# walaj/SeqLib

Measured on AMD Instinct MI355X. Metric: aligned reads/sec (150 bp) via BWAAligner, higher is better.
Workload: dtype int32

## Files before the change

### seqlib_amd/csrc/dev_fin.h

```cpp
#pragma once
#include "dev_ext.h"
#include "dev_as.h"

#define DEV_MINUS_INF (-0x40000000)

template <typename QF, typename TF>
__device__ int dev_ksw_global2(int qlen, QF qf, int tlen, TF tf, const slx_opt &o, int w, uint8_t *z, int n_col, int *eh_h, int *eh_e)
{
    const int8_t *mat = o.mat;
    const int o_del = o.o_del, e_del = o.e_del, o_ins = o.o_ins, e_ins = o.e_ins;
    const int oe_del = o_del + e_del, oe_ins = o_ins + e_ins;
    int i, j;
    eh_h[0] = 0; eh_e[0] = DEV_MINUS_INF;
    for (j = 1; j <= qlen && j <= w; ++j) { eh_h[j] = -(o_ins + e_ins * j); eh_e[j] = DEV_MINUS_INF; }
    for (; j <= qlen; ++j) eh_h[j] = eh_e[j] = DEV_MINUS_INF;
    for (i = 0; i < tlen; ++i) {
        int f = DEV_MINUS_INF, h1, beg, end, t;
        const int8_t *qrow = mat + tf(i) * 5;
        beg = i > w ? i - w : 0;
        end = i + w + 1 < qlen ? i + w + 1 : qlen;
        h1 = beg == 0 ? -(o_del + e_del * (i + 1)) : DEV_MINUS_INF;
        uint8_t *zi = z ? z + (size_t)i * n_col : nullptr;
        for (j = beg; j < end; ++j) {
            int h, m = eh_h[j], e = eh_e[j];
// ... 310 lines not shown
        const int64_t l_pac = rfl_i64(R.l_pac);
        SortStage S;
        S.idx = S.ka = S.kb = S.m_qe = S.m_rid = S.m_w = nullptr; S.k64 = S.m_rb = nullptr; S.nmax = 0; S.lane = 0;
        if (ss) {
            S.idx = lds_uniform(ss->idx); S.k64 = lds_uniform(ss->k64); S.ka = lds_uniform(ss->ka); S.kb = lds_uniform(ss->kb);
            S.m_rb = lds_uniform(ss->m_rb); S.m_qe = lds_uniform(ss->m_qe); S.m_rid = lds_uniform(ss->m_rid); S.m_w = lds_uniform(ss->m_w);
            S.nmax = rfl_i32(ss->nmax); S.lane = ss->lane;
            n = rfl_i32(n);
        }
        const bool staged = ss != nullptr && n <= S.nmax && n >= 2;
        glb_ptr<DReg> Gg = as_glb(G);
        glb_ptr<int> ag = as_glb(a);
        if (staged) { Gg = as_glb_uniform(G); ag = as_glb_uniform(a); }
        const bool dbg = ck.dbg_cyc && ck.dbg_stage == 2;
        unsigned long long t0 = dbg ? __builtin_readcyclecounter() : 0ull, t1 = t0, t2 = t0, t3 = t0;
        auto sort_handles = [&](int m, auto fill, auto less_lds, auto less_glb) {
            if (!staged) { ks_introsort_idx(m, a, less_glb); return; }
            __threadfence_block();
            for (int i = S.lane; i < m; i += 64) { const int h = ag[i]; S.idx[i] = h; fill(h); }
            fin_sync<MAXQ>();
            bool tie = m > 768;
            if (!tie) for (int e = S.lane; e < m; e += 64) {
                const int he = S.idx[e];
                int rank = 0;
                for (int j = 0; j < m; ++j) {
                    const int hj = S.idx[j];
                    const bool lt = less_lds(hj, he);
                    rank += lt ? 1 : 0;
                    if (!lt && j != e && !less_lds(he, hj)) tie = true;
                }
                S.m_w[e] = rank;
            }
            if (!__any(tie)) {
                fin_sync<MAXQ>();
                for (int e = S.lane; e < m; e += 64) S.m_rid[S.m_w[e]] = S.idx[e];
                fin_sync<MAXQ>();
                for (int e = S.lane; e < m; e += 64) { const int h = S.m_rid[e]; S.idx[e] = h; ag[e] = h; }
            } else {
                fin_sync<MAXQ>();
                if (S.lane == 0) ks_introsort_idx(m, S.idx, less_lds);
                fin_sync<MAXQ>();
                for (int i = S.lane; i < m; i += 64) ag[i] = S.idx[i];
            }
            fin_sync<MAXQ>();
            __threadfence_block();
        };
        if (staged) { for (int i = S.lane; i < n; i += 64) ag[i] = i; __threadfence_block(); }
        else for (int i = 0; i < n; ++i) a[i] = i;
        if (n > 1) {
            sort_handles(n, [&](int h) { S.k64[h] = Gg[h].re; },
                         [&](int x, int y) { return S.k64[x] < S.k64[y]; },
                         [&](int x, int y) { return G[x].re < G[y].re; });
            if (dbg) t1 = __builtin_readcyclecounter();
            if (defer && !staged && n <= 64) {
                for (int i = 1; i < n; ++i) {
                    const DReg &p = G[a[i]];
                    if (p.rid != G[a[i - 1]].rid || p.rb >= G[a[i - 1]].re + opt.max_chain_gap) continue;
                    for (int j = i - 1; j >= 0 && p.rid == G[a[j]].rid && p.rb < G[a[j]].re + opt.max_chain_gap; --j) {
                        const DReg &q = G[a[j]];
                        if (q.rb < p.rb && dev_patch_pre(R, opt, q.rb, q.re, q.qb, q.qe, q.w, p.rb, p.re, p.qb, p.qe, p.w) >= 0) { *defer = true; return -1; }
                    }
                }
            }
            if (staged) { for (int i = S.lane; i < n; i += 64) Gg[i].n_comp = 1; __threadfence_block(); }
            else for (int i = 0; i < n; ++i) G[a[i]].n_comp = 1;
// ... 111 lines not shown
                    const int i = base + S.lane;
                    const int h = i < n_in ? S.idx[i] : 0;
                    const bool keep = i < n_in && (i < first_forced || S.m_qe[h] > S.kb[h]);
                    const unsigned long long km = __ballot(keep);
                    const int pos = m + (int)__builtin_amdgcn_mbcnt_hi((uint32_t)(km >> 32), __builtin_amdgcn_mbcnt_lo((uint32_t)km, 0u));
                    if (keep) ag[pos] = h;
                    m += (int)__popcll(km);
                }
                __threadfence_block();
                return m;
            };
            int m = 0;
            if (staged) m = compact_staged(n, 0);
            else for (int i = 0; i < n; ++i) if (G[a[i]].qe > G[a[i]].qb) a[m++] = a[i];
            n = m;
            sort_handles(n, [&](int h) { S.ka[h] = Gg[h].score; S.k64[h] = Gg[h].rb; S.kb[h] = Gg[h].qb; },
                         [&](int x, int y) {
                             const int sx = S.ka[x], sy = S.ka[y];
                             const int64_t bx = S.k64[x], by = S.k64[y];
                             return sx > sy || (sx == sy && (bx < by || (bx == by && S.kb[x] < S.kb[y])));
                         },
                         [&](int x, int y) {
                             const DReg &X = G[x], &Y = G[y];
                             return X.score > Y.score || (X.score == Y.score && (X.rb < Y.rb || (X.rb == Y.rb && X.qb < Y.qb)));
                         });
            if (staged) {
                for (int i = 1 + S.lane; i < n; i += 64) {
                    const int h = S.idx[i], hp = S.idx[i - 1];
                    if (S.ka[h] == S.ka[hp] && S.k64[h] == S.k64[hp] && S.kb[h] == S.kb[hp]) { Gg[h].qe = S.kb[h]; S.m_qe[h] = S.kb[h]; }
                }
                fin_sync<MAXQ>();
// ... 65 lines not shown
                int n_pri = 0;
                for (int base = 0; base < n; base += 64) {
                    const int i = base + lane;
                    bool pri = false;
                    if (i < n) {
                        const int h = ag[i];
                        const glb_ptr<DReg> p = Gg + h;
                        p->sub = 0; p->secondary = -1; p->hash = dev_hash_64(id + (uint64_t)i);
                        const int al = ref_is_alt(R, p->rid);
                        l_alt[h] = al;
                        pri = !al;
                    }
                    n_pri += (int)__popcll(__ballot(pri));
                }
                __threadfence_block();
                sort_handles(n, [&](int h) { S.ka[h] = Gg[h].score; S.k64[h] = (int64_t)Gg[h].hash; },
                             [&](int x, int y) {
                                 const int sx = S.ka[x], sy = S.ka[y];
                                 if (sx != sy) return sx > sy;
                                 const int ax = l_alt[x], ay = l_alt[y];
                                 return ax < ay || (ax == ay && (uint64_t)S.k64[x] < (uint64_t)S.k64[y]);
                             },
                             [&](int x, int y) { return false; });
                core_staged(n, l_alt);
                if (n_pri < n) {
                    for (int i = lane; i < n; i += 64) { const int h = S.idx[i], sidx = Gg[h].secondary; l_par[h] = sidx >= 0 ? S.idx[sidx] : -1; }
                    fin_sync<MAXQ>();
                    if (n_pri > 0)
                        sort_handles(n, [&](int h) { S.ka[h] = Gg[h].score; S.k64[h] = (int64_t)Gg[h].hash; },
                                     [&](int x, int y) {
                                         const int ax = l_alt[x], ay = l_alt[y];
                                         if (ax != ay) return ax < ay;
                                         const int sx = S.ka[x], sy = S.ka[y];
                                         return sx > sy || (sx == sy && (uint64_t)S.k64[x] < (uint64_t)S.k64[y]);
                                     },
                                     [&](int x, int y) { return false; });
                    const lds_ptr<int> l_rank = (lds_ptr<int>)S.k64;
                    fin_sync<MAXQ>();
                    for (int i = lane; i < n; i += 64) l_rank[S.idx[i]] = i;
                    fin_sync<MAXQ>();
                    for (int i = lane; i < n; i += 64) {
                        const int h = S.idx[i], ph = l_par[h];
                        if (ph >= 0) { par[h] = l_rank[ph]; if (l_alt[h]) Gg[h].secondary = 0x7fffffff; }
                        else par[h] = -1;
// ... 5 lines not shown
                } else
                    for (int i = lane; i < n; i += 64) { const int h = S.idx[i]; par[h] = Gg[h].secondary; }
                __threadfence_block();
                fin_sync<MAXQ>();
            } else if (R.ann_alt) {
                dev_mark_primary_alt(R, opt, w, n, id);
            } else {
            if (staged) {
                for (int i = S.lane; i < n; i += 64) { const glb_ptr<DReg> p = Gg + ag[i]; p->sub = 0; p->secondary = -1; p->hash = dev_hash_64(id + (uint64_t)i); }
                __threadfence_block();
            } else for (int i = 0; i < n; ++i) {
                DReg &p = G[a[i]];
                p.sub = 0; p.secondary = -1;
                p.hash = dev_hash_64(id + (uint64_t)i);
            }
            sort_handles(n, [&](int h) { S.ka[h] = Gg[h].score; S.k64[h] = (int64_t)Gg[h].hash; },
                         [&](int x, int y) {
                             const int sx = S.ka[x], sy = S.ka[y];
                             return sx > sy || (sx == sy && (uint64_t)S.k64[x] < (uint64_t)S.k64[y]);
                         },
                         [&](int x, int y) {
                             const DReg &X = G[x], &Y = G[y];
                             return X.score > Y.score || (X.score == Y.score && X.hash < Y.hash);
                         });
            if (staged) core_staged(n, nullptr);
            else {
            int *z = w.ib, nz = 0;
            z[nz++] = 0;
            for (int i = 1; i < n; ++i) {
                int k;
                DReg &ai = G[a[i]];
// ... 67 lines not shown
```

### seqlib_amd/csrc/dev_fin2.h

```cpp
#pragma once
#include "dev_fin.h"
#include "dev_ext_reg.h"
#include "dev_nm8.h"

#ifndef LANE_CIG_BAND
#define LANE_CIG_BAND 33
#endif
#define LANE_CIG_MAXQ 158
#define LANE_CIG_MAXT 400
#define LANE_NEG (-16000)
#define LANE_FIN_LIMIT 8000
static_assert(LANE_NEG + LANE_FIN_LIMIT <= -LANE_FIN_LIMIT && LANE_NEG >= -32768 && LANE_FIN_LIMIT <= 32767, "16-bit cells of k_cig_lanes");
#define LANE_IL_WORDS(max_len) (((LANE_CIG_BAND + 3) / 4) * (((max_len) < LANE_CIG_MAXQ ? (max_len) : LANE_CIG_MAXQ) + 16))
struct alignas(8) DJob {
    int64_t rb, re;
    int qb, qe;
    int w2, truesc;
    int r, pad;
};

struct FinLists {
    DJob *jobs;
    uint32_t *fast_list, *dp_list;
    unsigned int *n_fast, *n_dp, *q_dp;
// ... 348 lines not shown
    __shared__ SortTables<NB> tables;
    const int lane = threadIdx.x;
    const SortStage ss = tables.stage(lane);
    const MatRows mr = make_matrows(dopt.o.mat);
    const int n_todo = __builtin_amdgcn_readfirstlane((int)*n_slots);
    for (;;) {
        const int slot = (int)wave_take(queue, 1u);
        if (slot >= n_todo) break;
        const int r = order ? order[slot] : slot;
        const int nr = __builtin_amdgcn_readfirstlane(ck.n_reg[r]);
        const bool mine = nr >= min_regs && nr <= max_regs;
        if (mine) dev_regs_read_wave<MAXQ>(R, ck, dopt.o, mr, fl, r, lane, &ss);
#ifdef REGS_SLEEP
        if (mine && nr >= 256) for (int t = 0; t < REGS_SLEEP; ++t) __builtin_amdgcn_s_sleep(127);
#endif
    }
}

__device__ __forceinline__ void dev_finish_hit(const DevRef &R, const Chunk &ck, const DJob &j, int l_query, DHit &h, int64_t cs, int nc)
{
    int is_rev;
    int64_t pos = dev_depos(R, j.rb < R.l_pac ? j.rb : j.re - 1, &is_rev);
    if (nc > 0) {
        if ((ck.cigpool[cs] & 0xf) == 2) { pos += ck.cigpool[cs] >> 4; ++cs; --nc; }
        else if ((ck.cigpool[cs + nc - 1] & 0xf) == 2) --nc;
    }
    if (j.qb != 0 || j.qe != l_query) {
        const int clip5 = is_rev ? l_query - j.qe : j.qb, clip3 = is_rev ? j.qb : l_query - j.qe;
        const uint32_t cop = ck.hardclip ? 5u : 4u;
        if (clip5) { --cs; ck.cigpool[cs] = (uint32_t)clip5 << 4 | cop; ++nc; }
// ... 253 lines not shown
    if (blockIdx.x < (n_jobs + CIG_BATCH - 1) / CIG_BATCH) {
        const unsigned long long off = wave_take_u64(ck.zused, (unsigned long long)CIG_WAVE_Z);
        if (off + CIG_WAVE_Z <= ck.zcap) { ws.z_own = ck.zarena + off; ws.z_own_cap = CIG_WAVE_Z; }
        else if (lane == 0) atomicOr(ck.flags + 1, OVS_Z_DP_WAVE);
    }
    for (;;) {
        const unsigned int t0 = wave_take(fl.q_dp, (unsigned int)CIG_BATCH);
        if (t0 >= n_jobs) break;
        const unsigned int t1 = t0 + CIG_BATCH < n_jobs ? t0 + CIG_BATCH : n_jobs;
        for (unsigned int t = t0; t < t1; ++t) dev_cig_dp_job<MAXQ>(R, ck, dopt.o, mr, fl, fl.dp_list[t], lane, ws);
    }
}

#define HITS_BIG 12
#define HITS_WAVE_N 2048
__global__ void __launch_bounds__(64) k_hits_wave(Chunk ck, const int *list, const unsigned int *n_list, unsigned int *queue)
{
    __shared__ int64_t s_pos[HITS_WAVE_N];
    __shared__ int s_rid[HITS_WAVE_N], s_mapq[HITS_WAVE_N];
    const int lane = threadIdx.x;
    const int n_todo = __builtin_amdgcn_readfirstlane((int)*n_list);
    for (;;) {
        const int slot = (int)wave_take(queue, 1u);
        if (slot >= n_todo) break;
        const int r = list[slot];
        ReadWS w = make_ws(ck, r);
        const int nh = __builtin_amdgcn_readfirstlane(ck.n_hit[r]);
        int *hh = w.ic;
        auto less_glb = [&](int x, int y) {
            const DHit &A = w.hits[x], &B = w.hits[y];
            if (A.mapq != B.mapq) return A.mapq > B.mapq;
            if (A.rid != B.rid) return A.rid < B.rid;
            return A.pos < B.pos;
        };
        bool serial = nh > HITS_WAVE_N;
        if (!serial) {
            __syncthreads();
            for (int e = lane; e < nh; e += 64) { const DHit &h = w.hits[e]; s_pos[e] = h.pos; s_rid[e] = h.rid; s_mapq[e] = h.mapq; }
            __syncthreads();
            bool tie = false;
            for (int base = 0; base < nh; base += 64) {
                const int e = base + lane;
                const bool live = e < nh;
                const int em = live ? s_mapq[e] : 0, er = live ? s_rid[e] : 0;
                const int64_t ep = live ? s_pos[e] : 0;
                int rank = 0;
                for (int j = 0; j < nh; ++j) {
                    const int jm = s_mapq[j], jr = s_rid[j];
                    const int64_t jp = s_pos[j];
                    const bool lt = jm != em ? jm > em : (jr != er ? jr < er : jp < ep);
                    rank += lt ? 1 : 0;
                    if (live && j != e && jm == em && jr == er && jp == ep) tie = true;
                }
                if (live) hh[rank] = e;
            }
            serial = __any(tie) != 0;
        }
        __threadfence_block();
        if (serial) {
            if (lane == 0) {
                for (int i = 0; i < nh; ++i) hh[i] = i;
                std_sort_idx(nh, hh, less_glb);
            }
            __threadfence_block();
        }
        __syncthreads();
        int n_out = 0;
        double carry = 0;
        for (int base = 0; base < nh; base += 64) {
            const int i = base + lane;
            const bool live = i < nh;
            const int hi = live ? hh[i] : 0;
            int flag = 0, score = 0;
// ... 115 lines not shown
```

### seqlib_amd/csrc/dev_types.h

```cpp
#pragma once
#include <hip/hip_runtime.h>
#include <stdint.h>
#include "seqlib_amd.h"
#include "dev_wave.h"

enum : uint32_t {
    OVF_INTV = 1u << 0,
    OVF_LIST = 1u << 1,
    OVF_ZARENA = 1u << 2,
    OVF_CIGAR = 1u << 3,
    ERR_LOGLUT = 1u << 4,
    ERR_INTERNAL = 1u << 5,
};
enum : uint32_t {
    OVS_Z_GEN = 1u << 8,
    OVS_Z_BAND = 1u << 9,
    OVS_Z_BAND_BLOCK = 1u << 10,
    OVS_Z_SEG = 1u << 11,
    OVS_Z_LANE = 1u << 12,
    OVS_Z_DP = 1u << 13,
    OVS_Z_DP_WAVE = 1u << 14,
    OVS_C_BAND = 1u << 15,
    OVS_C_LANE = 1u << 16,
    OVS_C_LONG = 1u << 17,
// ... 81 lines not shown
    int32_t *s_next;
    int32_t *s_score;
    int64_t *c_pos;
    int32_t *c_head, *c_tail, *c_n, *c_rid, *c_w, *c_first;
    int8_t *c_kept;
    int32_t *ia, *ib, *ic;
    uint64_t *srt;
    DReg *regs;
    DHit *hits;
    const DReg *cand;
    const int32_t *cand_base;
    unsigned long long *dbg_cyc;
    int dbg_stage;
    int ext_row_exit;
    unsigned int *ext_exits;
    int32_t *n_chain;
    int32_t *n_reg;
    int32_t *n_hit;
    int32_t *na;
    float *frac_rep;
    uint8_t *zarena; unsigned long long zcap; unsigned long long *zused;
    uint32_t *cigpool; unsigned long long cigcap; unsigned long long *cigused;
    const double *log_lut; int log_lut_n;
    uint32_t *flags;
    void *lists; int cap_list; int n_threads;
    int *long_scratch; int long_stride; int long_threads;
    int *huge_rows; int huge_stride;
    int hardclip; double keepSecFrac; int maxSecondary;
    int sam_mode;
};
// ... 54 lines not shown
```

### seqlib_amd/csrc/slx_align.hip

```cpp
#include <hip/hip_runtime.h>
#include <hipcub/hipcub.hpp>
#include <chrono>
#include <cmath>
#include <functional>
#include <unistd.h>
#include <cstdio>
#include <cstdlib>
#include <cstring>
#include <algorithm>
#include <mutex>
#include <string>
#include <thread>
#include <type_traits>
#include <vector>
#include "slx_internal.h"
#include "dev_seed4.h"
#include "dev_fin.h"
#include "dev_ext_wave.h"
#include "dev_ext_reg.h"
#include "dev_ext_lane.h"
#include "dev_ext_block.h"
#include "dev_ext_seg.h"
#include "dev_fin2.h"
#include "dev_chain_coop.h"
// ... 475 lines not shown
        while ((int)al->workers.size() < (int)value) { const int rc = add_worker(al); if (rc != SLX_OK) return rc; }
        al->n_workers = (int)value;
    }
    else if (!strcmp(key, "min_split")) { if (value < 1) return SLX_EINVAL; al->min_split = value; }
    else if (!strcmp(key, "seed_quota")) { if (value < 0 || value > (1 << 24)) return SLX_EINVAL; al->seed_quota = (int)value; }
    else if (!strcmp(key, "rep_k")) {
        if (value < 0 || value > 31) return SLX_EINVAL;
        al->rep_k = (int)value;
        HIPCHK(hipSetDevice(al->device));
        return al->wide ? build_rep_filter<uint64_t>(al) : build_rep_filter<uint32_t>(al);
    }
    else if (!strcmp(key, "top_heavy")) al->top_heavy = value != 0;
    else if (!strcmp(key, "top_reuse")) al->top_reuse = value != 0;
    else if (!strcmp(key, "walk_stage")) al->walk_stage = value != 0;
    else if (!strcmp(key, "ext_row_exit")) al->ext_row_exit = value != 0;
    else if (!strcmp(key, "ext_narrow")) { if (value < 0 || value > 3) return SLX_EINVAL; al->ext_narrow = (int)value; }
    else if (!strcmp(key, "p2_items")) al->p2_items = value != 0;
    else if (!strcmp(key, "p2_coop")) al->p2_coop = value != 0;
    else if (!strcmp(key, "p2_items_cap")) al->p2_items_cap = (int)value;
    else if (!strcmp(key, "seed_free_cus")) {
        if (value < 0 || value > 24) return SLX_EINVAL;
        HIPCHK(hipSetDevice(al->device));
        al->seed_free_cus = (int)value;
        for (Worker *wk : al->workers) { const int rc = set_seed_stream(al, wk); if (rc != SLX_OK) return rc; }
    }
    else if (!strcmp(key, "stream_prio")) {
        if (value < 0 || value > 1) return SLX_EINVAL;
        HIPCHK(hipSetDevice(al->device));
        al->stream_prio = (int)value;
        for (Worker *wk : al->workers) {
// ... 72 lines not shown
            long long v = 0;
            auto take = [&](const slx_aligner *a) { for (const Worker *wk : a->workers) v += (long long)wk->first_stat; };
            if (al->is_group) for (const slx_aligner *sub : al->subs) take(sub); else take(al);
            return v;
        }
        if (!strcmp(key, "ext_narrow_sides") || !strcmp(key, "ext_narrow_jobs")) {
            long long v = 0;
            const int which = key[11] == 'j';
            auto take = [&](const slx_aligner *a) { for (const Worker *wk : a->workers) v += (long long)wk->narrow_stat[which]; };
            if (al->is_group) for (const slx_aligner *sub : al->subs) take(sub); else take(al);
            return v;
        }
        if (!strcmp(key, "walk_staged_chains")) {
            long long v = 0;
            auto take = [&](const slx_aligner *a) { for (const Worker *wk : a->workers) v += (long long)wk->walk_stat; };
            if (al->is_group) for (const slx_aligner *sub : al->subs) take(sub); else take(al);
            return v;
        }
        if (!strcmp(key, "ext_row_exits")) {
            long long v = 0;
            auto take = [&](const slx_aligner *a) { for (const Worker *wk : a->workers) v += (long long)wk->exit_stat; };
            if (al->is_group) for (const slx_aligner *sub : al->subs) take(sub); else take(al);
            return v;
        }
        if (!strcmp(key, "retries")) {
            long long v = 0;
            if (al->is_group) for (const slx_aligner *sub : al->subs) v += sub->n_retries; else v = al->n_retries;
            return v;
        }
        if (!strcmp(key, "ovf_sites")) {
// ... 103 lines not shown
    if (h_offs && r_hi > r_lo) {
        const uint64_t b0 = h_offs[r_lo], b1 = h_offs[r_hi];
        if (b0 < al->h_first || b1 < b0 || b1 > al->h_last) { slx_set_error("read offsets are not monotonic (part [%lld, %lld))", (long long)r_lo, (long long)r_hi); return SLX_EINVAL; }
        if (b1 > b0) HIPCHK(hipMemcpyAsync((void *)(d_bases + b0), h_bases + b0, b1 - b0, hipMemcpyHostToDevice, wk->stream));
        HIPCHK(hipMemcpyAsync((void *)(d_offs + r_lo), h_offs + r_lo, ((size_t)(r_hi - r_lo) + 1) * 8, hipMemcpyHostToDevice, wk->stream));
    }
    for (int i = 0; i < SLX_N_STAGES; ++i) wk->stage_ms[i] = 0;
    for (int i = 0; i < SLX_N_PROBES; ++i) wk->probe_ms[i] = 0;
    wk->n_chunks = 0;
    for (long long &c : wk->cnt) c = 0;
    wk->chain_stat[0] = wk->chain_stat[1] = 0;
    wk->first_stat = 0;
    wk->walk_stat = 0;
    wk->exit_stat = 0;
    wk->narrow_stat[0] = wk->narrow_stat[1] = 0;
    int rc;
    const int64_t n_part = r_hi - r_lo;
    if ((rc = wk->o_hit_off.ensure(((size_t)n_part + 1) * 8)) != SLX_OK) return rc;
    if ((rc = wk->len_stat.ensure(32)) != SLX_OK) return rc;
    int64_t hit_base = 0, cig_base = 0;
    for (int64_t r0 = r_lo, step = 0; r0 < r_hi; r0 += step) {
        const int n = (int)std::min<int64_t>(al->chunk_reads, r_hi - r0);
        step = n;
        unsigned long long stat[4] = {0, 0, 0, 0};
        HIPCHK(hipMemsetAsync(wk->len_stat.p, 0, 32, wk->stream));
        hipLaunchKernelGGL(k_len_stats, dim3((unsigned)((n + 255) / 256)), dim3(256), 0, wk->stream, d_offs + r0, n, wk->len_stat.as<unsigned long long>());
        { MailSpec ms{}; ms.src[0] = wk->len_stat.as<unsigned int>(); ms.words[0] = 8; ms.n = 1;
          hipLaunchKernelGGL(k_mail, dim3(1), dim3(64), 0, wk->stream, ms, wk->h_mail); }
        HIPCHK(slx_wait_stream(wk->stream));
        memcpy(stat, wk->h_mail, 32);
// ... 581 lines not shown
```

### seqlib_amd/csrc/slx_align_types.h

```cpp
#pragma once
#include <hip/hip_runtime.h>
#include <mutex>
#include <string>
#include <vector>
#include "slx_internal.h"
#include "slx_hip.h"
#include "dev_fm.h"
#include "dev_types.h"

#define HIPCHK(x) SLX_HIPCHK(x)

struct DevBuf : SlxDevBuf<SlxMargin<8, 256>> {
    int grow(size_t bytes, size_t keep, hipStream_t st) { return bytes <= cap ? SLX_OK : slx_dev_realloc(&p, &cap, SlxMargin<2, 256>::want(bytes), st, keep); }
};

#define SLX_MAIL_PARTS 8
struct MailSpec { const unsigned int *src[SLX_MAIL_PARTS]; int words[SLX_MAIL_PARTS]; int n; };
static __global__ void k_mail(MailSpec s, unsigned int *dst)
{
    int at = 0;
    for (int i = 0; i < s.n; ++i) {
        for (int w = (int)threadIdx.x; w < s.words[i]; w += (int)blockDim.x) dst[at + w] = s.src[i][w];
        at += s.words[i];
    }
// ... 20 lines not shown
    DevBuf p2mask, p2list, p2items, p2long, lane_jobs, first_dp, cig_lane_list;
    DevBuf job_key_in, job_key_out, job_val_in, job_val_out, job_sort_tmp;
    DevBuf seed3_buf;
    DevBuf memo_idx, memo_jobs, memo_tab, round_list, todo_a, todo_b, spec_cnt;
    int long_rounds_run = 0; unsigned int long_jobs_run = 0;
    DevBuf xseg_jobs, xseg_state, xseg_units, xseg_out, xseg_wrec, xseg_wout, xseg_scratch, xseg_cnt;
    DevBuf gseg_jobs, gseg_units, gseg_wrec, gseg_wout, gseg_scratch, gseg_cnt;
    DevBuf pseg_jobs, pseg_idx, pseg_cnt;
    unsigned long long fin_stat[2] = {0, 0};
    unsigned long long chain_stat[2] = {0, 0};
    unsigned long long first_stat = 0;
    bool first_lanes_ran = false;
    unsigned long long walk_stat = 0;
    unsigned long long narrow_stat[2] = {0, 0};
    unsigned long long exit_stat = 0;
    unsigned int pseg_stat = 0;
    unsigned int gseg_stat[3] = {0, 0, 0};
    unsigned int xseg_stat[4] = {0, 0, 0, 0};
    DevBuf snap_ia, snap_regs, snap_nreg;
    Chunk last_ck;
    size_t last_S1 = 0;
    bool last_valid = false, last_wide = false;
    int id = 0;
    unsigned int max_seed_cnt = 0;
    hipEvent_t dbg_ev[6] = {nullptr, nullptr, nullptr, nullptr, nullptr, nullptr};
    DevBuf o_hit_off, o_rid, o_pos, o_flag, o_mapq, o_score, o_nm, o_na, o_ncig, o_cig_off, o_cigar, o_xa, o_sub;
    hipEvent_t ev[SLX_N_STAGES + 1];
    hipEvent_t ev_probe[6] = {nullptr, nullptr, nullptr, nullptr, nullptr, nullptr};
    float stage_ms[SLX_N_STAGES];
    float probe_ms[SLX_N_PROBES] = {0, 0, 0, 0, 0, 0};
// ... 74 lines not shown
    int cand_cap = 1 << 23;
    int lut_k = -1;
    int keep_stages = 0;
    int chain_mode = 1;
    int heavy_seeds = 64;
    int split_min = 4096;
    int seed_quota = 0;
    int top_heavy = 0;
    int p2_items = 1;
    int p2_coop = 1;
    int p2_items_cap = 0;
    int top_reuse = 1;
    int walk_stage = 1;
    int ext_row_exit = 1;
    int ext_narrow = 1;
    int seed_free_cus = 0;
    int stream_prio = 0;
    int n_workers = 3;
    int hw_queues = 4;
    int active_k = 1;
    int64_t min_split = 1 << 18;
    int max_threads = 0;
    int threads_per_cu = 1536;
    int n_cu = 256;
    unsigned long long zcap = 1ull << 26;
    unsigned long long z_per_read = 512;
    unsigned long long cig_per_read = 8;
    unsigned long long cig_floor = 0;
    int n_retries = 0;
    unsigned long long z_start = 0, cig_start = 0;
// ... 33 lines not shown
```

### seqlib_amd/csrc/slx_chunk.inc

```

__device__ __forceinline__ uint32_t nt4_of(uint32_t b)
{
    const uint32_t u = b & 0xDFu;
    const uint32_t x = (b >> 1) & 3u;
    const bool letter = u == 'A' || u == 'C' || u == 'G' || u == 'T';
    return b < 4u ? b : (letter ? (x ^ (x >> 1)) : 4u);
}

__global__ void k_encode(const uint8_t *ascii, uint8_t *codes, size_t n)
{
    const size_t n16 = (n + 15) >> 4;
    const size_t stride = (size_t)gridDim.x * blockDim.x;
    const bool aligned = ((uintptr_t)ascii & 3) == 0;
    for (size_t t = (size_t)blockIdx.x * blockDim.x + threadIdx.x; t < n16; t += stride) {
        const size_t i = t << 4;
        uint32_t w[4];
        if (aligned && i + 16 <= n) {
            const uint32_t *src = (const uint32_t *)(ascii + i);
#pragma unroll
            for (int k = 0; k < 4; ++k) w[k] = src[k];
        } else {
#pragma unroll
            for (int k = 0; k < 4; ++k) {
                w[k] = 0;
// ... 339 lines not shown
    hipLaunchKernelGGL(k_regs1, dim3(std::max(1, std::min(n / 256 + 1, al->n_cu * 8))), dim3(256), 0, st, ck, dopt, fl, wk->order_in.as<int>(), cnt2);
    int *multi = wk->order_out.as<int>();
    if constexpr (MAXQ <= 704) {
        if (al->regs_sorted && wk->order_bin.ensure((size_t)n * 4) == SLX_OK && wk->bin_cnt.ensure(512) == SLX_OK && hipMemsetAsync(wk->bin_cnt.p, 0, 512, st) == hipSuccess) {
            const dim3 gb((unsigned)((n + 255) / 256));
            unsigned int *bins = wk->bin_cnt.as<unsigned int>();
            hipLaunchKernelGGL(k_nreg_bin_count<int>, gb, dim3(256), 0, st, (const int *)wk->order_out.as<int>(), (const unsigned int *)(cnt2 + 1), (const int *)ck.n_reg, bins);
            hipLaunchKernelGGL(k_nreg_bin_scan, dim3(1), dim3(64), 0, st, bins);
            hipLaunchKernelGGL(k_nreg_bin_scatter<int>, gb, dim3(256), 0, st, (const int *)wk->order_out.as<int>(), (const unsigned int *)(cnt2 + 1), (const int *)ck.n_reg, bins, wk->order_bin.as<int>());
            multi = wk->order_bin.as<int>();
        } else (void)hipGetLastError();
    }
    if constexpr (MAXQ <= 704) {
        if (al->regs_big < (1 << 20)) {
            const int mid = std::max(al->regs_big, REGS_MID_N);
            if (al->regs_big <= REGS_MID_N)
                hipLaunchKernelGGL((k_regs_wave<MAXQ, REGS_MID_N>), dim3(std::max(1, std::min(n / 64 + 1, al->n_cu * 8))), dim3(64), 0, st, al->ref, ck, dopt, fl,
                                   multi, q + 11, cnt2 + 1, al->regs_big, REGS_MID_N);
            if (mid < 512 || wk->max_seed_cnt > (unsigned int)mid)
                hipLaunchKernelGGL((k_regs_wave<MAXQ, REGS_BIG_N>), dim3(std::max(1, std::min(n / 4096 + 1, al->n_cu))), dim3(64), 0, st, al->ref, ck, dopt, fl,
                                   multi, q + 15, cnt2 + 1, al->regs_big <= REGS_MID_N ? mid + 1 : al->regs_big, 1 << 30);
        }
        int *defer_list = (al->regs_defer && wk->defer_list.ensure((size_t)n * 4) == SLX_OK) ? wk->defer_list.as<int>() : nullptr;
        hipLaunchKernelGGL(k_regs<MAXQ>, dim3(ck.spread > 1 ? std::max(grid, (n + 1) / 2) : grid), dim3(bs), 0, st, al->ref, ck, dopt, fl, multi, q + 9, cnt2 + 1, ck.spread > 1 ? 1 : 0, al->regs_big,
                           defer_list, q + 46);
        if (defer_list)
            hipLaunchKernelGGL((k_regs_wave<MAXQ, REGS_SMALL_N>), dim3(std::max(1, std::min(n / 64 + 1, al->n_cu * 16))), dim3(64), 0, st, al->ref, ck, dopt, fl, (const int *)defer_list, q + 47,
                               (const unsigned int *)(q + 46), 0, 1 << 30);
    } else {
        unsigned int n_multi = 0;
        if (hipMemcpyAsync(&n_multi, cnt2 + 1, 4, hipMemcpyDeviceToHost, st) == hipSuccess && slx_wait_stream(st) == hipSuccess && n_multi > 1 &&
            wk->job_key_in.ensure((size_t)n_multi * 4) == SLX_OK && wk->job_val_in.ensure((size_t)n_multi * 4) == SLX_OK) {
            hipLaunchKernelGGL(k_read_len_keys, dim3((n_multi + 255) / 256), dim3(256), 0, st, ck.offs, (const int *)wk->order_out.as<int>(), n_multi, wk->job_key_in.as<unsigned int>(),
                               wk->job_val_in.as<unsigned int>());
            if (sort_keys_largest_first(wk, st, n_multi)) (void)hipMemcpyAsync(wk->order_out.p, wk->job_val_out.p, (size_t)n_multi * 4, hipMemcpyDeviceToDevice, st);
        }
// ... 160 lines not shown
    if (spread > 1) {
        seed_grid = std::max(seed_grid, (n + 1) / 2);
        n_threads = std::max(n_threads, seed_grid * bs);
    }
    const int cap_list = max_len + 1;
#define ENS(buf, bytes) if ((rc = wk->buf.ensure((size_t)(bytes))) != SLX_OK) return rc
    ENS(codes, n_bases + 16); ENS(offs_rel, ((size_t)n + 1) * 8);
    ENS(intv_n, (size_t)n * 4); ENS(intv_info, (size_t)n * caps.cap_intv * sizeof(qp_t)); ENS(intv_x0, (size_t)n * caps.cap_intv * sizeof(I));
    ENS(intv_x2, (size_t)n * caps.cap_intv * sizeof(I)); ENS(l_rep, (size_t)n * 4); ENS(seed_cnt, ((size_t)n + 1) * 8); ENS(seed_off, ((size_t)n + 1) * 8);
    ENS(n_chain, (size_t)n * 4); ENS(n_reg, (size_t)n * 4); ENS(n_hit, ((size_t)n + 1) * 4); ENS(na, (size_t)n * 4); ENS(frac_rep, (size_t)n * 4);
    ENS(lists, (size_t)2 * cap_list * n_threads * sizeof(IntvE<I>));
    ENS(zarena, caps.zcap); ENS(cigpool, caps.cigcap * 4);
    ENS(hit_cnt, ((size_t)n + 1) * 8); ENS(cig_cnt, ((size_t)n + 1) * 8); ENS(hit_off_c, ((size_t)n + 1) * 8); ENS(cig_off_c, ((size_t)n + 1) * 8);
    ENS(counters, 64); ENS(p2mask, (size_t)n * 8); ENS(p2list, (size_t)n * 4); ENS(p2items, (size_t)n * 4); ENS(p2long, (size_t)n * 4);
    HIPCHK(hipMemsetAsync(wk->counters.p, 0, 64, st));
    ENS(queues, 256);
    HIPCHK(hipMemsetAsync(wk->queues.p, 0, 256, st));
    wk->first_lanes_ran = false;
    HIPCHK(hipMemsetAsync(wk->seed_cnt.as<unsigned long long>() + n, 0, 8, st));

    Chunk ck;
    memset(&ck, 0, sizeof ck);
    ck.n_reads = n;
    ck.spread = spread;
    ck.codes = wk->codes.as<uint8_t>();
    ck.offs = wk->offs_rel.as<uint64_t>();
    ck.first_ordinal = first_ordinal + (uint64_t)r0;
    ck.rng_state = rng_state;
    ck.cap_intv = caps.cap_intv;
    ck.intv_n = wk->intv_n.as<uint32_t>(); ck.intv_info = wk->intv_info.as<uint32_t>();
    ck.intv_x0 = wk->intv_x0.p; ck.intv_x2 = wk->intv_x2.p;
    ck.l_rep = wk->l_rep.as<int32_t>();
    ck.seed_off = wk->seed_off.as<uint64_t>();
    ck.n_chain = wk->n_chain.as<int32_t>(); ck.n_reg = wk->n_reg.as<int32_t>(); ck.n_hit = wk->n_hit.as<int32_t>();
    ck.na = wk->na.as<int32_t>(); ck.frac_rep = wk->frac_rep.as<float>();
    ck.zarena = wk->zarena.as<uint8_t>(); ck.zcap = caps.zcap; ck.zused = wk->counters.as<unsigned long long>();
    ck.cigpool = wk->cigpool.as<uint32_t>(); ck.cigcap = caps.cigcap; ck.cigused = wk->counters.as<unsigned long long>() + 1;
    ck.flags = (uint32_t *)(wk->counters.as<unsigned long long>() + 2);
    ck.log_lut = al->d_loglut.as<double>(); ck.log_lut_n = SLX_LOG_LUT_N;
    ck.lists = wk->lists.p; ck.cap_list = cap_list; ck.n_threads = n_threads;
    ck.hardclip = hardclip; ck.keepSecFrac = ksf; ck.maxSecondary = maxsec;
    ck.sam_mode = (opt->flag & SLX_F_REG2SAM) ? 1 : 0;
    ck.seed_cnt = wk->seed_cnt.as<unsigned long long>();
    ck.ext_row_exit = al->ext_row_exit; ck.ext_exits = wk->queues.as<unsigned int>() + 56;
    const bool production = al->chain_mode == 1 && n >= al->split_min && !has_long;
    const bool use_cand = al->cand_mode == 1 && production;
    if (use_cand) {
        ENS(cand, (size_t)al->cand_cap * sizeof(DReg)); ENS(cand_base, (size_t)n * 4); ENS(cand_cnt, ((size_t)n + 2) * 8); ENS(cand_off, ((size_t)n + 2) * 8);
        HIPCHK(hipMemsetAsync(wk->cand_base.p, 0xff, (size_t)n * 4, st));
        ck.cand = wk->cand.as<DReg>(); ck.cand_base = wk->cand_base.as<int32_t>();
    }
    if (getenv("SLX_DEBUG_CYC")) {
        ENS(dbg_cyc, (size_t)n * 32);
        HIPCHK(hipMemsetAsync(wk->dbg_cyc.p, 0, (size_t)n * 32, st));
        ck.dbg_cyc = wk->dbg_cyc.as<unsigned long long>();
        ck.dbg_stage = atoi(getenv("SLX_DEBUG_CYC"));
    }
    DevOpt dopt; dopt.o = *opt;
    DevFM<I> fm = fm_of<I>(al);
// ... 345 lines not shown
    {
        MailSpec ms{};
        int at = 0;
        auto part = [&](const unsigned int *src, int words) {
            if (ms.n >= SLX_MAIL_PARTS || at + words > 64) return -1;
            ms.src[ms.n] = src; ms.words[ms.n] = words; ++ms.n;
            at += words;
            return at - words;
        };
        m_hits = part((const unsigned int *)(wk->hit_off_c.as<unsigned long long>() + n), 2);
        m_cig = part((const unsigned int *)(wk->cig_off_c.as<unsigned long long>() + n), 2);
        m_flags = part((const unsigned int *)ck.flags, 1);
        m_defer = part(wk->queues.as<unsigned int>() + 46, 1);
        m_big = part(wk->queues.as<unsigned int>() + 48, 1);
        m_chain = part(wk->queues.as<unsigned int>() + 50, 2);
        m_walk = part(wk->queues.as<unsigned int>() + 55, 5);
        if (wk->first_lanes_ran) m_first = part(wk->queues.as<unsigned int>() + 54, 1);
        if (m_hits < 0 || m_cig < 0 || m_flags < 0 || m_defer < 0 || m_big < 0 || m_chain < 0 || m_walk < 0 || (wk->first_lanes_ran && m_first < 0)) {
            slx_set_error("run_chunk: more counters than k_mail has parts (SLX_MAIL_PARTS)");
            return SLX_EINTERNAL;
        }
        hipLaunchKernelGGL(k_mail, dim3(1), dim3(64), 0, st, ms, wk->h_mail);
    }
    HIPCHK(slx_wait_stream(st));
    memcpy(&Hc, wk->h_mail + m_hits, 8); memcpy(&Cc, wk->h_mail + m_cig, 8);
    const uint32_t fl = wk->h_mail[m_flags];
    wk->fin_stat[0] += wk->h_mail[m_defer]; wk->fin_stat[1] += wk->h_mail[m_big];
    if (fl) { *flags_out = fl; return SLX_OK; }
    wk->chain_stat[0] += wk->h_mail[m_chain]; wk->chain_stat[1] += wk->h_mail[m_chain + 1];
    wk->walk_stat += wk->h_mail[m_walk];
    wk->exit_stat += wk->h_mail[m_walk + 1];
    wk->narrow_stat[0] += wk->h_mail[m_walk + 4]; wk->narrow_stat[1] += wk->h_mail[m_walk + 3];
    if (m_first >= 0) wk->first_stat += wk->h_mail[m_first];
    const size_t H = (size_t)*hit_base + Hc, C = (size_t)*cig_base + Cc;
#define GROW(buf, bytes, keep) if ((rc = wk->buf.grow((size_t)(bytes), (size_t)(keep), st)) != SLX_OK) return rc
    GROW(o_rid, (H + 1) * 4, *hit_base * 4); GROW(o_pos, (H + 1) * 8, *hit_base * 8); GROW(o_flag, (H + 1) * 2, *hit_base * 2);
    GROW(o_mapq, (H + 1), *hit_base); GROW(o_score, (H + 1) * 4, *hit_base * 4); GROW(o_nm, (H + 1) * 4, *hit_base * 4);
    GROW(o_na, (H + 1) * 4, *hit_base * 4); GROW(o_ncig, (H + 1) * 4, *hit_base * 4); GROW(o_cig_off, (H + 2) * 8, *hit_base * 8);
    GROW(o_cigar, (C + 1) * 4, *cig_base * 4);
    if (ck.sam_mode) { GROW(o_xa, (H + 1) * 4, *hit_base * 4); GROW(o_sub, (H + 1) * 4, *hit_base * 4); }
    HitsSoA so;
    so.hit_off = wk->o_hit_off.as<int64_t>(); so.rid = wk->o_rid.as<int32_t>(); so.pos = wk->o_pos.as<int64_t>();
    so.flag = wk->o_flag.as<uint16_t>(); so.mapq = wk->o_mapq.as<uint8_t>(); so.score = wk->o_score.as<int32_t>();
    so.nm = wk->o_nm.as<int32_t>(); so.na = wk->o_na.as<int32_t>(); so.n_cigar_ops = wk->o_ncig.as<int32_t>();
    so.cig_off = wk->o_cig_off.as<int64_t>(); so.cigar = wk->o_cigar.as<uint32_t>();
    so.xa_parent = ck.sam_mode ? wk->o_xa.as<int32_t>() : nullptr; so.sub = ck.sam_mode ? wk->o_sub.as<int32_t>() : nullptr;
    hipLaunchKernelGGL(k_compact, dim3((unsigned)((n + 255) / 256)), dim3(256), 0, st, ck, wk->hit_off_c.as<unsigned long long>(),
// ... 68 lines not shown
                    if (nrg[(size_t)i] >= lim[b] && (b == 5 || nrg[(size_t)i] < lim[b + 1])) {
                        ++cnt; cy += cyc[(size_t)i]; a += cyc[(size_t)n + i]; bb += cyc[2 * (size_t)n + i]; c += cyc[3 * (size_t)n + i];
                    }
                fprintf(stderr, "[regions >= %d] reads %ld  ticks %.3g (A %.3g B %.3g C %.3g)\n", lim[b], cnt, (double)cy, (double)a, (double)bb, (double)c);
            }
        }
        {
            const int lb[5] = {0, 1, 50, 100, 140};
            for (int b = 0; b < 5; ++b) {
                long cnt = 0; unsigned long long cy = 0;
                for (int i = 0; i < n; ++i)
                    if (nrg[(size_t)i] >= 256 && lrep[(size_t)i] >= lb[b] && (b == 4 || lrep[(size_t)i] < lb[b + 1])) { ++cnt; cy += cyc[(size_t)i]; }
                fprintf(stderr, "[>= 256 regions, l_rep >= %d] reads %ld  mean ticks %.3g\n", lb[b], cnt, cnt ? (double)cy / (double)cnt : 0.0);
            }
        }
        fprintf(stderr, "[ext cycles] n=%d total=%.3g (100 MHz ticks) heavy share=%.3f\n", n, (double)tot, tot ? (double)tot_heavy / (double)tot : 0.0);
        for (int i = 0; i < top; ++i) {
            const size_t r = (size_t)ord[(size_t)i];
            fprintf(stderr, "  read %zu: %.3g ticks (A %.3g, B %.3g, C %.3g; stage 1: sort, covered tests, extend+store; stage 2: sort by end, dedup/patch, second sort)  seeds=%llu chains=%d regions=%d l_rep=%d\n", r, (double)cyc[r],
                    (double)cyc[(size_t)n + r], (double)cyc[2 * (size_t)n + r], (double)cyc[3 * (size_t)n + r], sc[r], nch[r], nrg[r], lrep[r]);
        }
    }
    if (getenv("SLX_DEBUG_SUB")) {
        const char *nm[5] = {"chain", "extend", "regs", "cig", "hits"};
        fprintf(stderr, "[worker %d n=%d]", wk->id, n);
        for (int i = 0; i < 5; ++i) { float ms = -1; (void)hipEventElapsedTime(&ms, wk->dbg_ev[i], wk->dbg_ev[i + 1]); fprintf(stderr, " %s=%.1f", nm[i], ms); }
        float tot = -1; (void)hipEventElapsedTime(&tot, wk->dbg_ev[0], wk->dbg_ev[5]);
        fprintf(stderr, " total=%.1f\n", tot);
    }
    wk->last_ck = ck; wk->last_valid = true; wk->last_wide = sizeof(I) == 8;
// ... 8 lines not shown
```

Before: 80.01 million.

## Sort regions and hits with a wave-parallel bitonic network; prefilter region lists

Replaces the O(m^2) rank-counting sort in the staged finalization (and in the hits kernel) with a wave-wide bitonic sorting network over LDS handles for lists at or above a size threshold. On ties it falls back to the serial introsort. The change also adds a k_regs_pick kernel that splits reads into mid and big lists up front, so the wave region kernels stop scanning every multi-seed read. Adds counters for sort paths plus extra mail slots and queue space, at the cost of an extra launch and per-stage syncs.

After: 84.20 million (median of 6 runs). 5.2% higher.

```diff
diff --git a/seqlib_amd/csrc/dev_fin.h b/seqlib_amd/csrc/dev_fin.h
--- a/seqlib_amd/csrc/dev_fin.h
+++ b/seqlib_amd/csrc/dev_fin.h
@@ -1,8 +1,10 @@
 #pragma once
 #include "dev_ext.h"
 #include "dev_as.h"
+#include "dev_wave_sort.h"
 
 #define DEV_MINUS_INF (-0x40000000)
+#define SORT_NET_MIN 128
 
 template <typename QF, typename TF>
 __device__ int dev_ksw_global2(int qlen, QF qf, int tlen, TF tf, const slx_opt &o, int w, uint8_t *z, int n_col, int *eh_h, int *eh_e)
@@ -348,11 +350,34 @@
         if (staged) { Gg = as_glb_uniform(G); ag = as_glb_uniform(a); }
         const bool dbg = ck.dbg_cyc && ck.dbg_stage == 2;
         unsigned long long t0 = dbg ? __builtin_readcyclecounter() : 0ull, t1 = t0, t2 = t0, t3 = t0;
-        auto sort_handles = [&](int m, auto fill, auto less_lds, auto less_glb) {
+        auto sort_handles = [&](int m, bool first, auto fill, auto less_lds, auto less_glb) {
             if (!staged) { ks_introsort_idx(m, a, less_glb); return; }
             __threadfence_block();
             for (int i = S.lane; i < m; i += 64) { const int h = ag[i]; S.idx[i] = h; fill(h); }
             fin_sync<MAXQ>();
+            auto count = [&](bool serial) {
+                if (S.lane != 0 || !ck.sort_cnt) return;
+                atomicAdd(ck.sort_cnt + (serial ? 1 : 0), 1u);
+                if (serial && first) atomicAdd(ck.sort_cnt + 2, 1u);
+            };
+            if (ck.wave_sort && m >= (ck.wave_sort == 1 ? SORT_NET_MIN : 2)) {
+                const lds_ptr<int> idx = S.idx;
+                wave_sort(m, S.lane, [&](int i) { return idx[i]; }, [&](int i, int h) { idx[i] = h; }, less_lds, [] { fin_sync<MAXQ>(); });
+                const bool tie = __any(wave_sort_tie(m, S.lane, [&](int i) { return idx[i]; }, less_lds)) != 0;
+                count(tie);
+                if (!tie) for (int e = S.lane; e < m; e += 64) ag[e] = idx[e];
+                else {
+                    fin_sync<MAXQ>();
+                    for (int i = S.lane; i < m; i += 64) idx[i] = ag[i];
+                    fin_sync<MAXQ>();
+                    if (S.lane == 0) ks_introsort_idx(m, idx, less_lds);
+                    fin_sync<MAXQ>();
+                    for (int i = S.lane; i < m; i += 64) ag[i] = idx[i];
+                }
+                fin_sync<MAXQ>();
+                __threadfence_block();
+                return;
+            }
             bool tie = m > 768;
             if (!tie) for (int e = S.lane; e < m; e += 64) {
                 const int he = S.idx[e];
@@ -365,6 +390,7 @@
                 }
                 S.m_w[e] = rank;
             }
+            if (m >= 2) count(__any(tie) != 0);
             if (!__any(tie)) {
                 fin_sync<MAXQ>();
                 for (int e = S.lane; e < m; e += 64) S.m_rid[S.m_w[e]] = S.idx[e];
@@ -382,7 +408,7 @@
         if (staged) { for (int i = S.lane; i < n; i += 64) ag[i] = i; __threadfence_block(); }
         else for (int i = 0; i < n; ++i) a[i] = i;
         if (n > 1) {
-            sort_handles(n, [&](int h) { S.k64[h] = Gg[h].re; },
+            sort_handles(n, true, [&](int h) { S.k64[h] = Gg[h].re; },
                          [&](int x, int y) { return S.k64[x] < S.k64[y]; },
                          [&](int x, int y) { return G[x].re < G[y].re; });
             if (dbg) t1 = __builtin_readcyclecounter();
@@ -524,7 +550,7 @@
             if (staged) m = compact_staged(n, 0);
             else for (int i = 0; i < n; ++i) if (G[a[i]].qe > G[a[i]].qb) a[m++] = a[i];
             n = m;
-            sort_handles(n, [&](int h) { S.ka[h] = Gg[h].score; S.k64[h] = Gg[h].rb; S.kb[h] = Gg[h].qb; },
+            sort_handles(n, false, [&](int h) { S.ka[h] = Gg[h].score; S.k64[h] = Gg[h].rb; S.kb[h] = Gg[h].qb; },
                          [&](int x, int y) {
                              const int sx = S.ka[x], sy = S.ka[y];
                              const int64_t bx = S.k64[x], by = S.k64[y];
@@ -620,7 +646,7 @@
                     n_pri += (int)__popcll(__ballot(pri));
                 }
                 __threadfence_block();
-                sort_handles(n, [&](int h) { S.ka[h] = Gg[h].score; S.k64[h] = (int64_t)Gg[h].hash; },
+                sort_handles(n, false, [&](int h) { S.ka[h] = Gg[h].score; S.k64[h] = (int64_t)Gg[h].hash; },
                              [&](int x, int y) {
                                  const int sx = S.ka[x], sy = S.ka[y];
                                  if (sx != sy) return sx > sy;
@@ -633,7 +659,7 @@
                     for (int i = lane; i < n; i += 64) { const int h = S.idx[i], sidx = Gg[h].secondary; l_par[h] = sidx >= 0 ? S.idx[sidx] : -1; }
                     fin_sync<MAXQ>();
                     if (n_pri > 0)
-                        sort_handles(n, [&](int h) { S.ka[h] = Gg[h].score; S.k64[h] = (int64_t)Gg[h].hash; },
+                        sort_handles(n, false, [&](int h) { S.ka[h] = Gg[h].score; S.k64[h] = (int64_t)Gg[h].hash; },
                                      [&](int x, int y) {
                                          const int ax = l_alt[x], ay = l_alt[y];
                                          if (ax != ay) return ax < ay;
@@ -669,7 +695,7 @@
                 p.sub = 0; p.secondary = -1;
                 p.hash = dev_hash_64(id + (uint64_t)i);
             }
-            sort_handles(n, [&](int h) { S.ka[h] = Gg[h].score; S.k64[h] = (int64_t)Gg[h].hash; },
+            sort_handles(n, false, [&](int h) { S.ka[h] = Gg[h].score; S.k64[h] = (int64_t)Gg[h].hash; },
                          [&](int x, int y) {
                              const int sx = S.ka[x], sy = S.ka[y];
                              return sx > sy || (sx == sy && (uint64_t)S.k64[x] < (uint64_t)S.k64[y]);
diff --git a/seqlib_amd/csrc/dev_fin2.h b/seqlib_amd/csrc/dev_fin2.h
--- a/seqlib_amd/csrc/dev_fin2.h
+++ b/seqlib_amd/csrc/dev_fin2.h
@@ -386,6 +386,18 @@
 #ifdef REGS_SLEEP
         if (mine && nr >= 256) for (int t = 0; t < REGS_SLEEP; ++t) __builtin_amdgcn_s_sleep(127);
 #endif
+    }
+}
+
+__global__ void __launch_bounds__(256) k_regs_pick(const int *order, const unsigned int *n_slots, const int *n_reg, int lo, int mid, int *list_mid, unsigned int *n_mid,
+                                                   int *list_big, unsigned int *n_big)
+{
+    const unsigned int n = *n_slots;
+    for (unsigned int t = blockIdx.x * blockDim.x + threadIdx.x; t < n; t += gridDim.x * blockDim.x) {
+        const int r = order[t];
+        const int nr = n_reg[r];
+        if (nr >= lo && nr <= mid) list_mid[wave_fetch_inc(n_mid)] = r;
+        else if (nr > mid && nr >= lo) list_big[wave_fetch_inc(n_big)] = r;
     }
 }
 
@@ -669,6 +681,15 @@
 
 #define HITS_BIG 12
 #define HITS_WAVE_N 2048
+__device__ __forceinline__ bool dev_hit_less(int am, int ar, int64_t ap, int bm, int br, int64_t bp)
+{
+    if (am != bm) return am > bm;
+    if (ar != br) return ar < br;
+    return ap < bp;
+}
+struct HitKey { int64_t pos; int rid, mq_e; };
+#define HIT_KEY_SH 11
+static_assert(HITS_WAVE_N <= 1 << HIT_KEY_SH, "HitKey: the hit's number must fit below the mapq");
 __global__ void __launch_bounds__(64) k_hits_wave(Chunk ck, const int *list, const unsigned int *n_list, unsigned int *queue)
 {
     __shared__ int64_t s_pos[HITS_WAVE_N];
@@ -684,12 +705,20 @@
         int *hh = w.ic;
         auto less_glb = [&](int x, int y) {
             const DHit &A = w.hits[x], &B = w.hits[y];
-            if (A.mapq != B.mapq) return A.mapq > B.mapq;
-            if (A.rid != B.rid) return A.rid < B.rid;
-            return A.pos < B.pos;
+            return dev_hit_less(A.mapq, A.rid, A.pos, B.mapq, B.rid, B.pos);
         };
         bool serial = nh > HITS_WAVE_N;
-        if (!serial) {
+        if (!serial && ck.wave_sort && nh >= (ck.wave_sort == 1 ? SORT_NET_MIN : 2)) {
+            __syncthreads();
+            for (int e = lane; e < nh; e += 64) { const DHit &h = w.hits[e]; s_pos[e] = h.pos; s_rid[e] = h.rid; s_mapq[e] = (int)h.mapq << HIT_KEY_SH | e; }
+            __syncthreads();
+            auto load = [&](int i) { HitKey k; k.pos = s_pos[i]; k.rid = s_rid[i]; k.mq_e = s_mapq[i]; return k; };
+            auto store = [&](int i, const HitKey &k) { s_pos[i] = k.pos; s_rid[i] = k.rid; s_mapq[i] = k.mq_e; };
+            auto less = [](const HitKey &a, const HitKey &b) { return dev_hit_less(a.mq_e >> HIT_KEY_SH, a.rid, a.pos, b.mq_e >> HIT_KEY_SH, b.rid, b.pos); };
+            wave_sort(nh, lane, load, store, less, [] { __syncthreads(); });
+            serial = __any(wave_sort_tie(nh, lane, load, less)) != 0;
+            if (!serial) for (int e = lane; e < nh; e += 64) hh[e] = s_mapq[e] & ((1 << HIT_KEY_SH) - 1);
+        } else if (!serial) {
             __syncthreads();
             for (int e = lane; e < nh; e += 64) { const DHit &h = w.hits[e]; s_pos[e] = h.pos; s_rid[e] = h.rid; s_mapq[e] = h.mapq; }
             __syncthreads();
@@ -703,7 +732,7 @@
                 for (int j = 0; j < nh; ++j) {
                     const int jm = s_mapq[j], jr = s_rid[j];
                     const int64_t jp = s_pos[j];
-                    const bool lt = jm != em ? jm > em : (jr != er ? jr < er : jp < ep);
+                    const bool lt = dev_hit_less(jm, jr, jp, em, er, ep);
                     rank += lt ? 1 : 0;
                     if (live && j != e && jm == em && jr == er && jp == ep) tie = true;
                 }
@@ -712,6 +741,7 @@
             serial = __any(tie) != 0;
         }
         __threadfence_block();
+        if (lane == 0 && ck.sort_cnt) atomicAdd(ck.sort_cnt + (serial ? 6 : 5), 1u);
         if (serial) {
             if (lane == 0) {
                 for (int i = 0; i < nh; ++i) hh[i] = i;
diff --git a/seqlib_amd/csrc/dev_types.h b/seqlib_amd/csrc/dev_types.h
--- a/seqlib_amd/csrc/dev_types.h
+++ b/seqlib_amd/csrc/dev_types.h
@@ -119,6 +119,8 @@
     int dbg_stage;
     int ext_row_exit;
     unsigned int *ext_exits;
+    int wave_sort;
+    unsigned int *sort_cnt;
     int32_t *n_chain;
     int32_t *n_reg;
     int32_t *n_hit;
diff --git a/seqlib_amd/csrc/dev_wave_sort.h b/seqlib_amd/csrc/dev_wave_sort.h
--- /dev/null
+++ b/seqlib_amd/csrc/dev_wave_sort.h
@@ -0,0 +1,73 @@
+#pragma once
+#include <stdint.h>
+#if defined(__HIPCC__)
+#define WSORT_FN __host__ __device__ __forceinline__
+#else
+#define WSORT_FN static inline
+#endif
+
+#define WSORT_LANES 64
+#ifndef WSORT_UNROLL
+#define WSORT_UNROLL 4
+#endif
+
+struct WaveSortStage { int k, j; };
+
+WSORT_FN WaveSortStage wave_sort_begin() { WaveSortStage s; s.k = 1; s.j = 0; return s; }
+WSORT_FN bool wave_sort_next(int m, WaveSortStage &s)
+{
+    if (s.j > 1) { s.j >>= 1; return true; }
+    if (s.k >= m) return false;
+    s.k <<= 1; s.j = s.k >> 1;
+    return true;
+}
+
+template <typename LOAD, typename STORE, typename LESS>
+WSORT_FN void wave_sort_stage(int m, WaveSortStage s, int lane, LOAD load, STORE store, LESS less)
+{
+    const int j = s.j, two_j = j << 1;
+    const bool mirror = j == (s.k >> 1);
+    const int lj = 31 - __builtin_clz((unsigned)j);
+    typedef decltype(load(0)) V;
+    for (int t0 = lane;; t0 += WSORT_UNROLL * WSORT_LANES) {
+        int i[WSORT_UNROLL], p[WSORT_UNROLL];
+        bool on[WSORT_UNROLL], sw[WSORT_UNROLL];
+        V a[WSORT_UNROLL] = {}, b[WSORT_UNROLL] = {};
+#pragma unroll
+        for (int u = 0; u < WSORT_UNROLL; ++u) {
+            const int t = t0 + u * WSORT_LANES;
+            const int base = (t >> lj) * two_j, off = t & (j - 1);
+            i[u] = base + off;
+            p[u] = mirror ? base + two_j - 1 - off : i[u] + j;
+            on[u] = p[u] < m;
+        }
+        if (i[0] >= m) break;
+#pragma unroll
+        for (int u = 0; u < WSORT_UNROLL; ++u) if (on[u]) { a[u] = load(i[u]); b[u] = load(p[u]); }
+#pragma unroll
+        for (int u = 0; u < WSORT_UNROLL; ++u) sw[u] = on[u] && less(b[u], a[u]);
+#pragma unroll
+        for (int u = 0; u < WSORT_UNROLL; ++u) if (sw[u]) { store(i[u], b[u]); store(p[u], a[u]); }
+    }
+}
+
+template <typename LOAD, typename STORE, typename LESS, typename SYNC>
+WSORT_FN void wave_sort(int m, int lane, LOAD load, STORE store, LESS less, SYNC sync)
+{
+    for (WaveSortStage s = wave_sort_begin(); wave_sort_next(m, s);) {
+        wave_sort_stage(m, s, lane, load, store, less);
+        sync();
+    }
+}
+
+template <typename LOAD, typename LESS>
+WSORT_FN bool wave_sort_tie(int m, int lane, LOAD load, LESS less)
+{
+    bool tie = false;
+    for (int i = lane; i + 1 < m; i += WSORT_LANES) {
+        const auto a = load(i);
+        const auto b = load(i + 1);
+        if (!less(a, b) && !less(b, a)) tie = true;
+    }
+    return tie;
+}
diff --git a/seqlib_amd/csrc/slx_align.hip b/seqlib_amd/csrc/slx_align.hip
--- a/seqlib_amd/csrc/slx_align.hip
+++ b/seqlib_amd/csrc/slx_align.hip
@@ -513,6 +513,7 @@
     else if (!strcmp(key, "top_reuse")) al->top_reuse = value != 0;
     else if (!strcmp(key, "walk_stage")) al->walk_stage = value != 0;
     else if (!strcmp(key, "ext_row_exit")) al->ext_row_exit = value != 0;
+    else if (!strcmp(key, "wave_sort")) { if (value < 0 || value > 2) return SLX_EINVAL; al->wave_sort = (int)value; }
     else if (!strcmp(key, "ext_narrow")) { if (value < 0 || value > 3) return SLX_EINVAL; al->ext_narrow = (int)value; }
     else if (!strcmp(key, "p2_items")) al->p2_items = value != 0;
     else if (!strcmp(key, "p2_coop")) al->p2_coop = value != 0;
@@ -615,6 +616,15 @@
         if (!strcmp(key, "walk_staged_chains")) {
             long long v = 0;
             auto take = [&](const slx_aligner *a) { for (const Worker *wk : a->workers) v += (long long)wk->walk_stat; };
+            if (al->is_group) for (const slx_aligner *sub : al->subs) take(sub); else take(al);
+            return v;
+        }
+        static const char *const sort_keys[5] = {"sort_wave", "sort_serial", "sort_serial_re", "hits_sort_wave", "hits_sort_serial"};
+        int which = -1;
+        for (int i = 0; i < 5; ++i) if (!strcmp(key, sort_keys[i])) which = i;
+        if (which >= 0) {
+            long long v = 0;
+            auto take = [&](const slx_aligner *a) { for (const Worker *wk : a->workers) v += (long long)wk->sort_stat[which]; };
             if (al->is_group) for (const slx_aligner *sub : al->subs) take(sub); else take(al);
             return v;
         }
@@ -748,6 +758,7 @@
     wk->walk_stat = 0;
     wk->exit_stat = 0;
     wk->narrow_stat[0] = wk->narrow_stat[1] = 0;
+    for (unsigned long long &c : wk->sort_stat) c = 0;
     int rc;
     const int64_t n_part = r_hi - r_lo;
     if ((rc = wk->o_hit_off.ensure(((size_t)n_part + 1) * 8)) != SLX_OK) return rc;
diff --git a/seqlib_amd/csrc/slx_align_types.h b/seqlib_amd/csrc/slx_align_types.h
--- a/seqlib_amd/csrc/slx_align_types.h
+++ b/seqlib_amd/csrc/slx_align_types.h
@@ -58,6 +58,7 @@
     unsigned long long walk_stat = 0;
     unsigned long long narrow_stat[2] = {0, 0};
     unsigned long long exit_stat = 0;
+    unsigned long long sort_stat[5] = {0, 0, 0, 0, 0};
     unsigned int pseg_stat = 0;
     unsigned int gseg_stat[3] = {0, 0, 0};
     unsigned int xseg_stat[4] = {0, 0, 0, 0};
@@ -162,6 +163,7 @@
     int walk_stage = 1;
     int ext_row_exit = 1;
     int ext_narrow = 1;
+    int wave_sort = 1;
     int seed_free_cus = 0;
     int stream_prio = 0;
     int n_workers = 3;
diff --git a/seqlib_amd/csrc/slx_chunk.inc b/seqlib_amd/csrc/slx_chunk.inc
--- a/seqlib_amd/csrc/slx_chunk.inc
+++ b/seqlib_amd/csrc/slx_chunk.inc
@@ -377,12 +377,15 @@
     if constexpr (MAXQ <= 704) {
         if (al->regs_big < (1 << 20)) {
             const int mid = std::max(al->regs_big, REGS_MID_N);
+            int *list_mid = wk->part_flag.as<int>(), *list_big = wk->part_pos.as<int>();
+            hipLaunchKernelGGL(k_regs_pick, dim3(std::max(1, std::min(n / 256 + 1, al->n_cu * 8))), dim3(256), 0, st, (const int *)multi, (const unsigned int *)(cnt2 + 1), (const int *)ck.n_reg,
+                               al->regs_big, al->regs_big <= REGS_MID_N ? REGS_MID_N : al->regs_big - 1, list_mid, q + 64, list_big, q + 65);
             if (al->regs_big <= REGS_MID_N)
                 hipLaunchKernelGGL((k_regs_wave<MAXQ, REGS_MID_N>), dim3(std::max(1, std::min(n / 64 + 1, al->n_cu * 8))), dim3(64), 0, st, al->ref, ck, dopt, fl,
-                                   multi, q + 11, cnt2 + 1, al->regs_big, REGS_MID_N);
+                                   (const int *)list_mid, q + 11, (const unsigned int *)(q + 64), al->regs_big, REGS_MID_N);
             if (mid < 512 || wk->max_seed_cnt > (unsigned int)mid)
                 hipLaunchKernelGGL((k_regs_wave<MAXQ, REGS_BIG_N>), dim3(std::max(1, std::min(n / 4096 + 1, al->n_cu))), dim3(64), 0, st, al->ref, ck, dopt, fl,
-                                   multi, q + 15, cnt2 + 1, al->regs_big <= REGS_MID_N ? mid + 1 : al->regs_big, 1 << 30);
+                                   (const int *)list_big, q + 15, (const unsigned int *)(q + 65), al->regs_big <= REGS_MID_N ? mid + 1 : al->regs_big, 1 << 30);
         }
         int *defer_list = (al->regs_defer && wk->defer_list.ensure((size_t)n * 4) == SLX_OK) ? wk->defer_list.as<int>() : nullptr;
         hipLaunchKernelGGL(k_regs<MAXQ>, dim3(ck.spread > 1 ? std::max(grid, (n + 1) / 2) : grid), dim3(bs), 0, st, al->ref, ck, dopt, fl, multi, q + 9, cnt2 + 1, ck.spread > 1 ? 1 : 0, al->regs_big,
@@ -573,8 +576,8 @@
     ENS(hit_cnt, ((size_t)n + 1) * 8); ENS(cig_cnt, ((size_t)n + 1) * 8); ENS(hit_off_c, ((size_t)n + 1) * 8); ENS(cig_off_c, ((size_t)n + 1) * 8);
     ENS(counters, 64); ENS(p2mask, (size_t)n * 8); ENS(p2list, (size_t)n * 4); ENS(p2items, (size_t)n * 4); ENS(p2long, (size_t)n * 4);
     HIPCHK(hipMemsetAsync(wk->counters.p, 0, 64, st));
-    ENS(queues, 256);
-    HIPCHK(hipMemsetAsync(wk->queues.p, 0, 256, st));
+    ENS(queues, 320);
+    HIPCHK(hipMemsetAsync(wk->queues.p, 0, 320, st));
     wk->first_lanes_ran = false;
     HIPCHK(hipMemsetAsync(wk->seed_cnt.as<unsigned long long>() + n, 0, 8, st));
 
@@ -602,6 +605,7 @@
     ck.sam_mode = (opt->flag & SLX_F_REG2SAM) ? 1 : 0;
     ck.seed_cnt = wk->seed_cnt.as<unsigned long long>();
     ck.ext_row_exit = al->ext_row_exit; ck.ext_exits = wk->queues.as<unsigned int>() + 56;
+    ck.wave_sort = al->wave_sort; ck.sort_cnt = wk->queues.as<unsigned int>() + 61;
     const bool production = al->chain_mode == 1 && n >= al->split_min && !has_long;
     const bool use_cand = al->cand_mode == 1 && production;
     if (use_cand) {
@@ -977,7 +981,7 @@
         m_defer = part(wk->queues.as<unsigned int>() + 46, 1);
         m_big = part(wk->queues.as<unsigned int>() + 48, 1);
         m_chain = part(wk->queues.as<unsigned int>() + 50, 2);
-        m_walk = part(wk->queues.as<unsigned int>() + 55, 5);
+        m_walk = part(wk->queues.as<unsigned int>() + 55, 13);
         if (wk->first_lanes_ran) m_first = part(wk->queues.as<unsigned int>() + 54, 1);
         if (m_hits < 0 || m_cig < 0 || m_flags < 0 || m_defer < 0 || m_big < 0 || m_chain < 0 || m_walk < 0 || (wk->first_lanes_ran && m_first < 0)) {
             slx_set_error("run_chunk: more counters than k_mail has parts (SLX_MAIL_PARTS)");
@@ -994,6 +998,8 @@
     wk->walk_stat += wk->h_mail[m_walk];
     wk->exit_stat += wk->h_mail[m_walk + 1];
     wk->narrow_stat[0] += wk->h_mail[m_walk + 4]; wk->narrow_stat[1] += wk->h_mail[m_walk + 3];
+    for (int i = 0; i < 3; ++i) wk->sort_stat[i] += wk->h_mail[m_walk + 6 + i];
+    wk->sort_stat[3] += wk->h_mail[m_walk + 11]; wk->sort_stat[4] += wk->h_mail[m_walk + 12];
     if (m_first >= 0) wk->first_stat += wk->h_mail[m_first];
     const size_t H = (size_t)*hit_base + Hc, C = (size_t)*cig_base + Cc;
 #define GROW(buf, bytes, keep) if ((rc = wk->buf.grow((size_t)(bytes), (size_t)(keep), st)) != SLX_OK) return rc
@@ -1092,6 +1098,9 @@
                 fprintf(stderr, "[>= 256 regions, l_rep >= %d] reads %ld  mean ticks %.3g\n", lb[b], cnt, cnt ? (double)cy / (double)cnt : 0.0);
             }
         }
+        if (ck.dbg_stage == 2)
+            fprintf(stderr, "[region sorts] wave_sort %d: on the wave %llu, one lane %llu (of those by region end %llu)\n", al->wave_sort, (unsigned long long)wk->h_mail[m_walk + 6],
+                    (unsigned long long)wk->h_mail[m_walk + 7], (unsigned long long)wk->h_mail[m_walk + 8]);
         fprintf(stderr, "[ext cycles] n=%d total=%.3g (100 MHz ticks) heavy share=%.3f\n", n, (double)tot, tot ? (double)tot_heavy / (double)tot : 0.0);
         for (int i = 0; i < top; ++i) {
             const size_t r = (size_t)ord[(size_t)i];
```
